# HUBioDataLab/DrugGEN

Hardware: AMD Instinct MI355X
Metric: molecules/sec GAN step (G+D fwd+bwd), N=45 graphs (higher is better)
Workload: dtype f32

## Files before the change

### druggen_amd/csrc/edge_ffn.hip

```cpp
#include "bf16.h"

using namespace dg;

extern "C" size_t dg_edge_ffn_ln_workspace_bytes(int64_t R, int C, int H) {
    const size_t ln = dg_ln_workspace_bytes(R, C);
    const size_t w1 = dg_linear_wgrad_workspace_bytes(R, H, C), w2 = dg_linear_wgrad_workspace_bytes(R, C, H);
    if (!ln || !w1 || !w2) return 0;
    return ((ln + 255) / 256 + (w1 + 255) / 256 + (w2 + 255) / 256) * 256;
}

extern "C" int dg_edge_ffn_ln_fwd(const void* x, const void* w1_packed, const float* b1, const void* w2_packed,
                                  const float* b2, const float* gamma, const float* beta, void* y, void* h,
                                  unsigned* relu_bits, void* pre_ln, float* mean, float* rstd, int64_t R, int C,
                                  int H, float eps, int dtype, dg_stream_t stream) {
    if (!x || !w1_packed || !b1 || !w2_packed || !b2 || !gamma || !beta || !y || !h || !mean || !rstd)
        return fail(DG_E_ARG, "dg_edge_ffn_ln_fwd: null pointer");
    if (C != 128 || H != 384) return fail(DG_E_SHAPE, "dg_edge_ffn_ln_fwd: needs dim 128, hidden 384 (got %d, %d)", C, H);
    int st = dg_row_gemm(x, w1_packed, h, R, C, H, b1, 1, relu_bits, nullptr, nullptr, nullptr, nullptr, nullptr,
                         nullptr, nullptr, 0.f, dtype, stream);
    if (st) return st;
    return dg_row_gemm(h, w2_packed, y, R, H, C, b2, 0, nullptr, nullptr, x, gamma, beta, mean, rstd, pre_ln, eps,
                       dtype, stream);
}

extern "C" int dg_edge_ffn_ln_bwd(const void* x, const void* h, const unsigned* relu_bits, const void* pre_ln,
                                  const float* mean, const float* rstd, const float* gamma,
                                  const void* w1_dgrad_packed, const void* w2_dgrad_packed, const void* dy,
                                  const void* dz_add, void* dz, void* dh, void* dx, float* dgamma, float* dbeta, float* dw1,
                                  float* db1, float* dw2, float* db2, void* workspace, size_t workspace_bytes,
                                  int64_t R, int C, int H, int dtype, dg_stream_t stream) {
    if (!x || !h || !relu_bits || !pre_ln || !mean || !rstd || !gamma || !w1_dgrad_packed || !w2_dgrad_packed ||
        !dz || !dh || !workspace)
        return fail(DG_E_ARG, "dg_edge_ffn_ln_bwd: null pointer");
    if (!dy && dz_add != dz)
        return fail(DG_E_ARG, "dg_edge_ffn_ln_bwd: dy == NULL means dz already holds the LayerNorm input gradient (pass it as dz_add too)");
    if (C != 128 || H != 384) return fail(DG_E_SHAPE, "dg_edge_ffn_ln_bwd: needs dim 128, hidden 384 (got %d, %d)", C, H);
    if (workspace_bytes < dg_edge_ffn_ln_workspace_bytes(R, C, H))
        return fail(DG_E_WORKSPACE, "dg_edge_ffn_ln_bwd: workspace too small");
    int st = 0;
    const size_t lnb = (dg_ln_workspace_bytes(R, C) + 255) / 256 * 256;
    const bool batch = dw2 && dw1;
    if (batch) dg_linear_wgrad_batch_begin();
    if (dy)
        st = dg_ln_residual_bwd_add(pre_ln, nullptr, gamma, mean, rstd, dy, dz_add, dz, dgamma, dbeta, workspace,
                                    lnb, R, C, act_dtype(dtype), stream);
    if (st) {
        if (batch) dg_linear_wgrad_batch_end(stream);
        return st;
    }
    workspace = static_cast<char*>(workspace) + lnb;
    workspace_bytes -= lnb;
    const int dt_h = ffn_h_dtype(dtype), dt_dh = ffn_dh_dtype(dtype);
    st = dg_row_gemm(dz, w2_dgrad_packed, dh, R, C, H, nullptr, 0, nullptr, relu_bits, nullptr, nullptr, nullptr,
                     nullptr, nullptr, nullptr, 0.f, dt_dh, stream);
    if (!st && dx)
        st = dg_row_gemm(dh, w1_dgrad_packed, dx, R, H, C, nullptr, 0, nullptr, nullptr, dz, nullptr, nullptr,
                         nullptr, nullptr, nullptr, 0.f, dt_dh, stream);
    if (st) {
        if (batch) dg_linear_wgrad_batch_end(stream);
        return st;
    }
    if (batch) {
        const size_t w2b = (dg_linear_wgrad_workspace_bytes(R, C, H) + 255) / 256 * 256;
        st = dg_linear_wgrad(dz, nullptr, h, dw2, db2, workspace, w2b, R, C, H, dt_h, stream);
        if (!st)
            st = dg_linear_wgrad(dh, nullptr, x, dw1, db1, static_cast<char*>(workspace) + w2b, workspace_bytes - w2b, R, H, C,
                                 dt_dh, stream);
        const int st2 = dg_linear_wgrad_batch_end(stream);
        return st ? st : st2;
    }
    if (dw2) {
        st = dg_linear_wgrad(dz, nullptr, h, dw2, db2, workspace, workspace_bytes, R, C, H, dt_h, stream);
        if (st) return st;
    }
    if (dw1) {
        st = dg_linear_wgrad(dh, nullptr, x, dw1, db1, workspace, workspace_bytes, R, H, C, dt_dh, stream);
        if (st) return st;
    }
    return 0;
}

namespace {

int ffn_fwd_check(const dg_ffn_fwd_args* a, const char* who) {
    if (!a || !a->x || !a->w1_packed || !a->b1 || !a->w2_packed || !a->b2 || !a->gamma || !a->beta || !a->y || !a->h ||
        !a->mean || !a->rstd)
        return fail(DG_E_ARG, "dg_edge_ffn_ln_fwd_pair: null pointer (%s)", who);
    return 0;
}

int ffn_bwd_phase(const dg_ffn_bwd_args& a, int phase, int C, int H, int dtype, dg_stream_t stream) {
    const int64_t R = a.R;
    const size_t lnb = (dg_ln_workspace_bytes(R, C) + 255) / 256 * 256;
    const size_t w2b = (dg_linear_wgrad_workspace_bytes(R, C, H) + 255) / 256 * 256;
    char* ws = static_cast<char*>(a.workspace);
    switch (phase) {
        case 0:
            if (!a.dy) return 0;
            return dg_ln_residual_bwd_add(a.pre_ln, nullptr, a.gamma, a.mean, a.rstd, a.dy, a.dz_add, a.dz, a.dgamma, a.dbeta, ws,
                                          lnb, R, C, act_dtype(dtype), stream);
        case 1:
            return dg_row_gemm(a.dz, a.w2_dgrad_packed, a.dh, R, C, H, nullptr, 0, nullptr, a.relu_bits, nullptr, nullptr,
                               nullptr, nullptr, nullptr, nullptr, 0.f, ffn_dh_dtype(dtype), stream);
        case 2:
            if (!a.dx) return 0;
            return dg_row_gemm(a.dh, a.w1_dgrad_packed, a.dx, R, H, C, nullptr, 0, nullptr, nullptr, a.dz, nullptr, nullptr,
                               nullptr, nullptr, nullptr, 0.f, ffn_dh_dtype(dtype), stream);
        case 3:
            if (!a.dw2) return 0;
            return dg_linear_wgrad(a.dz, nullptr, a.h, a.dw2, a.db2, ws + lnb, w2b, R, C, H, ffn_h_dtype(dtype), stream);
        default:
            if (!a.dw1) return 0;
            return dg_linear_wgrad(a.dh, nullptr, a.x, a.dw1, a.db1, ws + lnb + w2b, a.workspace_bytes - lnb - w2b, R, H, C,
                                   ffn_dh_dtype(dtype), stream);
    }
}

}

extern "C" int dg_edge_ffn_ln_fwd_pair(const dg_ffn_fwd_args* node, const dg_ffn_fwd_args* edge, int C, int H, int dtype,
                                       dg_stream_t stream) {
    if (int st = ffn_fwd_check(node, "node")) return st;
    if (int st = ffn_fwd_check(edge, "edge")) return st;
    if (C != 128 || H != 384) return fail(DG_E_SHAPE, "dg_edge_ffn_ln_fwd_pair: needs dim 128, hidden 384 (got %d, %d)", C, H);
    const dg_ffn_fwd_args* ps[2] = {node, edge};
    dg_launch_pair_begin();
    int st = 0;
    for (int i = 0; i < 2 && !st; ++i)
        st = dg_row_gemm(ps[i]->x, ps[i]->w1_packed, ps[i]->h, ps[i]->R, C, H, ps[i]->b1, 1, ps[i]->relu_bits, nullptr, nullptr,
                         nullptr, nullptr, nullptr, nullptr, nullptr, 0.f, dtype, stream);
    for (int i = 0; i < 2 && !st; ++i)
        st = dg_row_gemm(ps[i]->h, ps[i]->w2_packed, ps[i]->y, ps[i]->R, H, C, ps[i]->b2, 0, nullptr, nullptr, ps[i]->x,
                         ps[i]->gamma, ps[i]->beta, ps[i]->mean, ps[i]->rstd, ps[i]->pre_ln, ps[i]->eps, dtype, stream);
    const int st2 = dg_launch_pair_end(stream);
    return st ? st : st2;
}

extern "C" int dg_edge_ffn_ln_bwd_pair(const dg_ffn_bwd_args* node, const dg_ffn_bwd_args* edge, int C, int H, int dtype,
                                       dg_stream_t stream) {
    const dg_ffn_bwd_args* ps[2] = {node, edge};
    for (const dg_ffn_bwd_args* a : ps) {
        if (!a || !a->x || !a->h || !a->relu_bits || !a->pre_ln || !a->mean || !a->rstd || !a->gamma || !a->w1_dgrad_packed ||
            !a->w2_dgrad_packed || !a->dz || !a->dh || !a->workspace)
            return fail(DG_E_ARG, "dg_edge_ffn_ln_bwd_pair: null pointer");
        if (!a->dy && a->dz_add != a->dz)
            return fail(DG_E_ARG, "dg_edge_ffn_ln_bwd_pair: dy == NULL means dz already holds the LayerNorm input gradient (pass it as dz_add too)");
        if (a->workspace_bytes < dg_edge_ffn_ln_workspace_bytes(a->R, C, H))
            return fail(DG_E_WORKSPACE, "dg_edge_ffn_ln_bwd_pair: workspace too small");
    }
    if (C != 128 || H != 384) return fail(DG_E_SHAPE, "dg_edge_ffn_ln_bwd_pair: needs dim 128, hidden 384 (got %d, %d)", C, H);
    dg_linear_wgrad_batch_begin();
    dg_launch_pair_begin();
    int st = 0;
    for (int phase = 0; phase < 5 && !st; ++phase)
        for (int i = 0; i < 2 && !st; ++i) st = ffn_bwd_phase(*ps[i], phase, C, H, dtype, stream);
    const int st2 = dg_launch_pair_end(stream);
    const int st3 = dg_linear_wgrad_batch_end(stream);
    return st ? st : (st2 ? st2 : st3);
}
```

### druggen_amd/csrc/row_gemm.hip

```cpp
#include "common.h"
#include "f16_scale.h"
#include "lane_reduce.h"
#include "row_gemm_n384.h"
#include "row_gemm_k384.h"
#include "traversal.h"

#include <cstring>
#include <type_traits>

#ifndef DG_DBG
#define DG_DBG 0
#endif
namespace dg {
namespace {

typedef float f32x16 __attribute__((ext_vector_type(16)));

constexpr int kTR = 64;

struct Epilogue {
    const float* bias;
    const unsigned* mask_bits;
    unsigned* relu_bits;
    const float* residual;
// ... 1117 lines not shown
    return check_launch("dg_row_gemm_ln_bwd");
}

bool reduce_batch_try_add(const float* part, int S, long long n_floats, float* out);

int row_gemm_f32_ln_in(const float* dy, const float* pre, const float* mean, const float* rstd, const float* gamma,
                       const float* packed, float* dz, float* y, float* dgamma, float* dbeta, void* workspace,
                       size_t workspace_bytes, int64_t R, dg_stream_t stream_) {
    if (!dy || !pre || !mean || !rstd || !gamma || !packed || !dz || !y || !workspace)
        return fail(DG_E_ARG, "dg_row_gemm_ln_bwd_in: null pointer");
    if (R < 0) return fail(DG_E_SHAPE, "dg_row_gemm_ln_bwd_in: R = %lld", static_cast<long long>(R));
    if (workspace_bytes < row_gemm_f32_ln_bwd_workspace_bytes()) return fail(DG_E_WORKSPACE, "dg_row_gemm_ln_bwd_in: workspace too small");
    if (R == 0) return 0;
    hipStream_t stream = static_cast<hipStream_t>(stream_);
    Epilogue ep{nullptr, nullptr, nullptr, nullptr, gamma, nullptr, const_cast<float*>(mean), const_cast<float*>(rstd), nullptr, 0.f, 0};
    ep.lna_pre = pre;
    ep.lna_dz = dz;
    ep.lnb_part = static_cast<float*>(workspace);
    const int64_t tiles = (R + kTR - 1) / kTR;
    const int seqs = static_cast<int>(tiles < 256 ? tiles : 256);
    {
        ProfScope prof(R < edge_rows() ? DG_K_ROW_GEMM : DG_K_ROW_GEMM_E_128, stream);
        note_forward(R);
        constexpr int lds = kH3Lds + 4 * 32 * 32 * 4;
        DG_OPT_IN_LDS((&row_gemm_h3_kernel<1, false, false, true>), lds);
        hipLaunchKernelGGL((row_gemm_h3_kernel<1, false, false, true>), dim3(seqs), dim3(512), lds, stream, dy,
                           reinterpret_cast<const f16x8*>(packed), y, R, ep);
    }
    if ((dgamma || dbeta) && !(dgamma && dbeta == dgamma + 128 && reduce_batch_try_add(ep.lnb_part, seqs * 8, 256, dgamma)))
        launch_ln_finish(ep.lnb_part, seqs * 8, 2, 128, dgamma, dbeta, stream);
    return check_launch("dg_row_gemm_ln_bwd_in");
}


int row_gemm_f32_lin3(const float* a, const float* packed, float* y0, float* y1, float* y2, int64_t R, const float* b0,
                      const float* b1, const float* b2, dg_stream_t stream_) {
    if (!a || !packed || !y0 || !y1 || !y2) return fail(DG_E_ARG, "dg_row_gemm_lin3: null pointer");
    if (R < 0) return fail(DG_E_SHAPE, "dg_row_gemm_lin3: negative row count");
    if (R == 0) return 0;
    hipStream_t stream = static_cast<hipStream_t>(stream_);
    Epilogue ep{b0, nullptr, nullptr, nullptr, nullptr, nullptr, nullptr, nullptr, nullptr, 0.f, 0};
    ep.y_alt[0] = y1;
    ep.y_alt[1] = y2;
    ep.bias_alt[0] = b1;
    ep.bias_alt[1] = b2;
    const int64_t tiles = (R + kTR - 1) / kTR;
    const int seqs = static_cast<int>(tiles < 256 ? tiles : 256);
    ProfScope prof(R < edge_rows() ? DG_K_ROW_GEMM : DG_K_ROW_GEMM_E_N384, stream);
    constexpr int lds3 = kH3Lds + 4 * 32 * 32 * 4;
    DG_OPT_IN_LDS((&row_gemm_h3_kernel<3, false, false, false, true>), lds3);
    hipLaunchKernelGGL((row_gemm_h3_kernel<3, false, false, false, true>), dim3(seqs), dim3(512), lds3, stream, a,
                       reinterpret_cast<const f16x8*>(packed), y0, R, ep);
    return check_launch("dg_row_gemm_lin3");
}

int row_gemm_f32_sum3(const float* a0, const float* a1, const float* a2, const float* packed, float* y, int64_t R,
                      const float* residual, dg_stream_t stream_) {
    if (!a0 || !a1 || !a2 || !packed || !y) return fail(DG_E_ARG, "dg_row_gemm_sum3: null pointer");
    if (R < 0) return fail(DG_E_SHAPE, "dg_row_gemm_sum3: negative row count");
    if (R == 0) return 0;
    hipStream_t stream = static_cast<hipStream_t>(stream_);
    Epilogue ep{nullptr, nullptr, nullptr, residual, nullptr, nullptr, nullptr, nullptr, nullptr, 0.f, 0};
    ep.a_alt[0] = a1;
    ep.a_alt[1] = a2;
    const int64_t tiles = (R + kTR - 1) / kTR;
    const int seqs = static_cast<int>(tiles < 256 ? tiles : 256);
// ... 16 lines not shown
```

### druggen_amd/csrc/row_gemm_n384.h

```cpp
#pragma once

#include "common.h"

namespace dg {

size_t row_gemm_n384_mask_words(int64_t R);
int launch_row_gemm_n384(const float* a, const void* packed, void* y, float* yscale, int64_t R, const float* bias, int relu,
                         unsigned* relu_bits, const unsigned* mask_bits, hipStream_t stream, int yfmt = 0, void* ylo = nullptr);
int flush_row_gemm_n384(hipStream_t stream);

}
```

### druggen_amd/csrc/row_gemm_n384.hip

```cpp
#include "common.h"

#include <cstdlib>
#include "row_gemm_n384.h"
#include "lane_reduce.h"
#include "f16_scale.h"
#include "pair.h"
#include "traversal.h"

#ifndef N3_SCHED
#define N3_SCHED 1
#endif
#ifndef N3_DBG
#define N3_DBG 0
#endif
namespace dg {
namespace {

constexpr int kSR = 32;
constexpr int kPlane = 16 * 512;
constexpr int kStage = 2 * kPlane + 128;
constexpr int kOut = kSR * 96 * 16;
constexpr int kOffOut = 2 * kStage;
constexpr int kOffTab = kOffOut + 2 * kOut;
constexpr int kOffBitsIn = kOffTab + 2 * 384 * 4;
constexpr int kOffBitsOut = kOffBitsIn + 2 * 2048;
constexpr int kLds = kOffBitsOut + 2 * 2048;
constexpr int kCons = 8, kProd = 4, kDepth = 3;

struct Epi {
    const float* bias;
    const unsigned* mask_bits;
    unsigned* relu_bits;
    int relu;
    int reverse;
};

struct Prob {
    const float* a;
    const f16x8* packed;
    float* y;
    float* yscale;
    void* ylo;
    int yfmt;
    int64_t R;
    Epi ep;
};

template <int FMT, int MODE, int NP = 3>
__global__ __launch_bounds__(64 * (kCons + kProd)) void row_gemm_n384_kernel(const Prob p0, const Prob p1, const int nb0) {
    constexpr bool H16 = FMT == 1 || FMT == 3, TWO = FMT == 3, H24 = FMT == 2;
    static_assert(NP == 3 || ((NP == 1 || NP == 2) && FMT == 1 && MODE == 2), "reduced products: fp16-plane results of the backward only");
    extern __shared__ __attribute__((aligned(16))) char smem[];
    float* const tab = reinterpret_cast<float*>(smem + kOffTab);
    const int lane = threadIdx.x & 63;
    const int w = __builtin_amdgcn_readfirstlane(threadIdx.x >> 6);
    const bool second = static_cast<int>(blockIdx.x) >= nb0;
    const float* __restrict__ const a = second ? p1.a : p0.a;
    const f16x8* __restrict__ const packed = second ? p1.packed : p0.packed;
    float* __restrict__ const y = second ? p1.y : p0.y;
    float* __restrict__ const yscale = second ? p1.yscale : p0.yscale;
    void* __restrict__ const ylo = second ? p1.ylo : p0.ylo;
    const int64_t R = second ? p1.R : p0.R;
    const Epi ep = second ? p1.ep : p0.ep;
    const int bidx = second ? static_cast<int>(blockIdx.x) - nb0 : static_cast<int>(blockIdx.x);
    const int nblk = second ? static_cast<int>(gridDim.x) - nb0 : nb0;
    const int64_t total = (R + kSR - 1) / kSR;
    const int T = static_cast<int>((total - bidx + nblk - 1) / nblk);
    auto stage_of = [&](int t) {
        const int64_t st = bidx + static_cast<int64_t>(t) * nblk;
        return ep.reverse ? total - 1 - st : st;
    };
    const int TP = (T + kDepth - 1) / kDepth * kDepth;

    if (w >= kCons) {
        __builtin_amdgcn_s_setprio(3);
        const int pt = threadIdx.x - 64 * kCons;
        const int hw = pt >> 5, l32 = pt & 31;
        {
            const float* inv_cs = reinterpret_cast<const float*>(packed + static_cast<size_t>(12) * 8 * 2 * 64);
            for (int i = pt; i < 384; i += 64 * kProd) {
                tab[i] = inv_cs[i];
                tab[384 + i] = ep.bias ? ep.bias[i] : 0.f;
            }
        }
        float4 pf[kDepth][4];
        u32x2 mk[kDepth];
        const unsigned voff = static_cast<unsigned>(hw) * 512u + static_cast<unsigned>(l32) * 16u;
        auto fetch = [&](float4 (&set)[4], u32x2& mword, int t) {
            if (t > T - 1) t = T - 1;
            const __amdgpu_buffer_rsrc_t rmask = __builtin_amdgcn_make_buffer_rsrc(
                const_cast<unsigned*>(ep.mask_bits ? ep.mask_bits + stage_of(t) * 512 : reinterpret_cast<const unsigned*>(a)), 0,
                ep.mask_bits ? 2048 : 0, 0x00020000);
            mword = __builtin_amdgcn_raw_buffer_load_b64(rmask, static_cast<unsigned>(pt) * 8u, 0, 0);
            const int64_t r0 = stage_of(t) * kSR;
            const int64_t left = (R - r0) * 512;
            const __amdgpu_buffer_rsrc_t rsrc = __builtin_amdgcn_make_buffer_rsrc(
                const_cast<float*>(a) + r0 * 128, 0, static_cast<int>(left < (1 << 30) ? left : (1 << 30)), 0x00020000);
            if (N3_DBG & 8) return;
#pragma unroll
            for (int i = 0; i < 4; ++i)
                set[i] = __builtin_bit_cast(float4, __builtin_amdgcn_raw_buffer_load_b128(rsrc, voff, i * 4096, 0));
        };
        const int blk = l32 >> 1;
        const unsigned wbase = static_cast<unsigned>(blk * 512 + (l32 & 1) * 8);
        auto split = [&](float4 (&set)[4], const u32x2& mword, int t) {
// ... 118 lines not shown
                const int64_t left = (R - r0) * 1152;
                const int bytes = ok ? static_cast<int>(left < kSR * 1152 ? left : kSR * 1152) : 0;
                const __amdgpu_buffer_rsrc_t rsrc = __builtin_amdgcn_make_buffer_rsrc(reinterpret_cast<char*>(y) + r0 * 1152, 0, bytes, 0x00020000);
                const unsigned g24 = static_cast<unsigned>(hw) * 1152u + static_cast<unsigned>(l32 ^ hw) * 12u;
                dg_u32x3 pk[12];
#pragma unroll
                for (int i = 0; i < 12; ++i) {
                    const int k = i / 3, qq = i % 3;
                    const float4 v = *reinterpret_cast<const float4*>(ot + ooff + k * 8 * 1536 + qq * 512);
                    pk[i] = pack_f24x4(v.x, v.y, v.z, v.w);
                }
                asm volatile("" : "+v"(pk[0]), "+v"(pk[1]), "+v"(pk[2]), "+v"(pk[3]), "+v"(pk[4]), "+v"(pk[5]), "+v"(pk[6]), "+v"(pk[7]),
                             "+v"(pk[8]), "+v"(pk[9]), "+v"(pk[10]), "+v"(pk[11]));
#pragma unroll
                for (int i = 0; i < 12; ++i) __builtin_amdgcn_raw_buffer_store_b96(pk[i], rsrc, g24, (i / 3) * 8 * 1152 + (i % 3) * 384, 0);
                asm volatile("s_nop 15" ::: "memory");
            } else {
                const int64_t left = (R - r0) * 1536;
                const int bytes = ok ? static_cast<int>(left < kSR * 1536 ? left : kSR * 1536) : 0;
                const __amdgpu_buffer_rsrc_t rsrc = __builtin_amdgcn_make_buffer_rsrc(y + r0 * 384, 0, bytes, 0x00020000);
#pragma unroll
                for (int i = 0; i < 12; ++i) {
                    const int k = i / 3, qq = i % 3;
                    const u32x4 v = *reinterpret_cast<const u32x4*>(ot + ooff + k * 8 * 1536 + qq * 512);
                    __builtin_amdgcn_raw_buffer_store_b128(v, rsrc, goff, k * 8 * 1536 + qq * 512, 0);
                }
            }
            const __amdgpu_buffer_rsrc_t rbits = __builtin_amdgcn_make_buffer_rsrc(
                ep.relu_bits ? ep.relu_bits + stage_of(tc) * 512 : reinterpret_cast<unsigned*>(y), 0, (ok && ep.relu_bits) ? 2048 : 0,
                0x00020000);
            const u32x2 bw = *reinterpret_cast<const u32x2*>(smem + kOffBitsOut + (tc & 1) * 2048 + pt * 8);
            __builtin_amdgcn_raw_buffer_store_b64(bw, rbits, static_cast<unsigned>(pt) * 8u, 0, 0);
        };
        fetch(pf[0], mk[0], 0);
        fetch(pf[1], mk[1], 1);
        fetch(pf[2], mk[2], 2);
        split(pf[0], mk[0], 0);
        fetch(pf[0], mk[0], 3);
        __syncthreads();
        for (int t = 0; t < TP; t += 3) {
            split(pf[1], mk[1], t + 1);
            fetch(pf[1], mk[1], t + 4);
            store_out(t - 1);
            __syncthreads();
            split(pf[2], mk[2], t + 2);
            fetch(pf[2], mk[2], t + 5);
            store_out(t);
            __syncthreads();
            split(pf[0], mk[0], t + 3);
            fetch(pf[0], mk[0], t + 6);
            store_out(t + 1);
            __syncthreads();
        }
        store_out(TP - 1);
        return;
    }

    const int n = lane & 15, kq = lane >> 4;
    f16x8 wf[3][4][NP == 1 ? 1 : 2];
#pragma unroll
    for (int cb = 0; cb < 3; ++cb) {
        const int ch = 48 * w + 16 * cb + n;
        const int tslab = ch >> 5, col = ch & 31;
#pragma unroll
        for (int ks = 0; ks < 4; ++ks)
#pragma unroll
// ... 79 lines not shown
                            newbits |= (v[i] > 0.f ? 1u : 0u) << bit;
                            v[i] = __uint_as_float((__float_as_uint(fmaxf(v[i], 0.f)) & relu_sel) | (__float_as_uint(v[i]) & ~relu_sel));
                            v[i] = (bits >> bit) & 1u ? v[i] : 0.f;
                        }
                    }
                    const int slot = (c0 >> 2) ^ (row & 7);
                    *reinterpret_cast<float4*>(ot + row * 1536 + slot * 16) = make_float4(v[0], v[1], v[2], v[3]);
                }
            }
            *reinterpret_cast<unsigned*>(smem + kOffBitsOut + (t & 1) * 2048 + (w * 64 + lane) * 4) = newbits;
        }
        __syncthreads();
    }
}

}

size_t row_gemm_n384_mask_words(int64_t R) { return static_cast<size_t>((R + kSR - 1) / kSR) * kCons * 64; }

namespace {
struct Pending {
    bool valid = false;
    Prob p;
};
thread_local Pending g_rider;

int mode_of(const Prob& p) {
    if (p.ep.relu && !p.ep.mask_bits) return 1;
    if (!p.ep.relu && p.ep.mask_bits && !p.ep.relu_bits && !p.ep.bias) return 2;
    return 0;
}
bool same_kernel(const Prob& a, const Prob& b) { return a.yfmt == b.yfmt && mode_of(a) == mode_of(b); }

int launch(const Prob& p0, const Prob* p1, hipStream_t stream) {
    const int64_t st0 = (p0.R + kSR - 1) / kSR, st1 = p1 ? (p1->R + kSR - 1) / kSR : 0;
    int nb0, nb1;
    pair_split(st0, st1, 256, &nb0, &nb1);
    const int mode = mode_of(p0);
#define DG_N384_LAUNCH(H16_, MODE_)                                                                                     \
    {                                                                                                                    \
        DG_OPT_IN_LDS((&row_gemm_n384_kernel<H16_, MODE_>), kLds);                                                       \
        hipLaunchKernelGGL((row_gemm_n384_kernel<H16_, MODE_>), dim3(nb0 + nb1), dim3(64 * (kCons + kProd)), kLds, stream, p0, \
                           p1 ? *p1 : p0, nb0);                                                                          \
    }
    const int dh_products = 2;
    if (p0.yfmt == 1) {
        if (mode == 1) DG_N384_LAUNCH(1, 1)
        else if (mode == 2 && dh_products == 2) {
            DG_OPT_IN_LDS((&row_gemm_n384_kernel<1, 2, 2>), kLds);
            hipLaunchKernelGGL((row_gemm_n384_kernel<1, 2, 2>), dim3(nb0 + nb1), dim3(64 * (kCons + kProd)), kLds, stream, p0,
                               p1 ? *p1 : p0, nb0);
        } else if (mode == 2 && dh_products == 1) {
            DG_OPT_IN_LDS((&row_gemm_n384_kernel<1, 2, 1>), kLds);
            hipLaunchKernelGGL((row_gemm_n384_kernel<1, 2, 1>), dim3(nb0 + nb1), dim3(64 * (kCons + kProd)), kLds, stream, p0,
                               p1 ? *p1 : p0, nb0);
        } else if (mode == 2) DG_N384_LAUNCH(1, 2)
        else DG_N384_LAUNCH(1, 0)
    } else if (p0.yfmt == 3) {
        if (mode == 1) DG_N384_LAUNCH(3, 1)
        else if (mode == 2) DG_N384_LAUNCH(3, 2)
        else DG_N384_LAUNCH(3, 0)
    } else if (p0.yfmt == 2) {
        if (mode == 1) DG_N384_LAUNCH(2, 1)
        else if (mode == 2) DG_N384_LAUNCH(2, 2)
        else DG_N384_LAUNCH(2, 0)
    } else {
        if (mode == 1) DG_N384_LAUNCH(0, 1)
        else if (mode == 2) DG_N384_LAUNCH(0, 2)
        else DG_N384_LAUNCH(0, 0)
    }
#undef DG_N384_LAUNCH
    return 0;
}
}

int flush_row_gemm_n384(hipStream_t stream) {
    if (!g_rider.valid) return 0;
    g_rider.valid = false;
    return launch(g_rider.p, nullptr, stream);
}

int launch_row_gemm_n384(const float* a, const void* packed, void* y, float* yscale, int64_t R, const float* bias, int relu,
                         unsigned* relu_bits, const unsigned* mask_bits, hipStream_t stream, int yfmt, void* ylo) {
    if ((yfmt == 1 || yfmt == 3) != (yscale != nullptr)) return fail(DG_E_ARG, "row_gemm_n384: row scales go with the fp16 planes (yfmt 1, 3)");
    if ((yfmt == 3) != (ylo != nullptr)) return fail(DG_E_ARG, "row_gemm_n384: the lo plane goes with yfmt 3");
    const Prob p{a, static_cast<const f16x8*>(packed), static_cast<float*>(y), yscale, ylo, yfmt, R,
                 Epi{bias, mask_bits, relu_bits, relu, take_direction(R)}};
    if (pair_mode() && !g_rider.valid && R <= kRiderMaxRows) {
        g_rider.valid = true;
        g_rider.p = p;
        return 0;
    }
    if (g_rider.valid) {
        g_rider.valid = false;
        if (same_kernel(p, g_rider.p)) return launch(p, &g_rider.p, stream);
        if (int st = launch(g_rider.p, nullptr, stream)) return st;
    }
    return launch(p, nullptr, stream);
}

}
```

### druggen_amd/functional/_runtime.py

```python
from __future__ import annotations

import contextlib
import threading
import weakref

import torch

from .. import _lib
from ..options import options


_traffic = {}


def traffic_reset() -> None:
    _traffic.clear()


def traffic_bytes(kernel: str) -> int:
    return _traffic.get(kernel, 0)


def _account(kernel: str, nbytes: int, flops: int = 0, floor: int = -1) -> None:
    _traffic[kernel] = _traffic.get(kernel, 0) + nbytes
# ... 60 lines not shown
    if adt == torch.float32:
        mode = hidden_storage()
        if mode in ("f16", "f24"):
            return _lib.F32_H16 if mode == "f16" else _lib.F32_H24
        if hidden_forward_storage(long_rows) == "split":
            return _lib.F32_H32
    return _lib.DTYPES[adt]


def _hidden_code_bwd(adt) -> int:
    if adt == torch.float32:
        mode = hidden_storage()
        if mode in ("f16", "dh16"):
            return _lib.F32_H16
        if mode in ("f24", "dh24"):
            return _lib.F32_H24
    return _lib.DTYPES[adt]


def _ffn_bwd_codes(h, adt, R: int, H: int):
    if _is_h16(h):
        code = _hidden_code_of(h, R, H)
        if code == _lib.F32_H32:
            return _lib.F32_H32_DH16, _lib.F32_H16
        return code, code
    dh_code = _hidden_code_bwd(adt)
    if dh_code == _lib.F32_H16 and hidden_storage() == "dh16":
        dh_code = _lib.F32_H24
    if dh_code == _lib.F32_H16:
        return _lib.F32_DH16, dh_code
    if dh_code == _lib.F32_H24:
        return _lib.F32_DH24, dh_code
    return _lib.DTYPES[adt], _lib.DTYPES[adt]


def _hidden_empty(R: int, H: int, adt, code: int, device):
    if code in _lib.HIDDEN_CODES:
        return torch.empty(int(_lib.load().dg_hidden_bytes(R, H, code)), dtype=torch.uint8, device=device)
    return torch.empty(R, H, dtype=adt, device=device)


def _hrow_bytes(code: int, es: int, H: int) -> int:
    if code == _lib.F32_H32:
        return 4 * H + 4
    return 2 * H + 4 if code == _lib.F32_H16 else (3 * H if code == _lib.F32_H24 else es * H)


def _is_h16(t) -> bool:
    return t is not None and t.dtype == torch.uint8


def _hptr(t):
    return t.data_ptr() if _is_h16(t) else _lib.ptr(t)


def _hidden_code_of(buf, R: int, H: int = 384) -> int:
    if buf.numel() == R * H * 3:
        return _lib.F32_H24
    plane = (R * H * 2 + 255) // 256 * 256
    return _lib.F32_H32 if buf.numel() == 2 * plane + 4 * R else _lib.F32_H16


def hidden_to_float(buf, R: int, H: int = 384):
    if _hidden_code_of(buf, R, H) == _lib.F32_H24:
        b = buf.view(R * H, 3).to(torch.int32)
        bits = (b[:, 0] << 8) | (b[:, 1] << 16) | (b[:, 2] << 24)
# ... 239 lines not shown
```

### druggen_amd/functional/ffn.py

```python
from __future__ import annotations

import ctypes

import torch
from torch.autograd import Function
from torch.autograd.function import once_differentiable

from .. import _lib
from ..options import options
from ._runtime import (_account, _alias_outputs_enabled, _c, _ffn_bwd_codes, _gemm_key, _hidden_code, _hidden_code_of,
                       _hidden_empty, hidden_storage, _hptr, _hrow_bytes, in_second_order_forward, _inputs_only, _is_h16,
                       _long_rows, PackCache, _pair_launches, _scratch, _weight_alias, _wgrad_key)
from .layernorm import ln_residual
from .dense import _double_backward_fallback, _join_alias_grads, linear, _ln_bwd2_rows, packed_weight, row_gemm, _wgrad_many


def _fused_ffn_enabled() -> bool:
    return options.ffn_bf16 == "fused"


def _composite_ffn_ln(x, w1, b1, w2, b2, gamma, beta, eps):
    return ln_residual(x, linear(torch.relu(linear(x, w1, b1)), w2, b2), gamma, beta, eps)


_ffn_f32_pack_cache = PackCache(1024)


def _ffn_packed_f32(w1, w2):
    def make(w1, w2):
        lib = _lib.load()
        packed = torch.empty(int(lib.dg_ffn_f32_packed_bytes()), dtype=torch.uint8, device=w1.device)
        _lib.launch("dg_ffn_f32_pack", w1, _lib.fptr(_c(w1.detach())), _lib.fptr(_c(w2.detach())), packed.data_ptr())
        return packed
    return _ffn_f32_pack_cache.get((w1, w2), (), make)


def set_fused_ffn_f32(on: bool) -> None:
    options.ffn_f32 = "fused" if on else "unfused"


def fused_ffn_f32_supported(x2, w1, w2, long_rows: bool = False) -> bool:
    return (options.ffn_f32 == "fused" and x2.is_cuda and x2.dtype == torch.float32 and tuple(w1.shape) == (384, 128)
            and tuple(w2.shape) == (128, 384) and hidden_storage() == "dh16" and not long_rows)
# ... 62 lines not shown
    return probs


def _ffn_saved(args, p):
    return (*args, p["h"], p["mean"], p["rstd"], p["pre"], p["bits"])


def _ffn_bwd_inputs(saved, needs, dy, dpre):
    x, w1, b1, w2, b2, gamma, beta, h, mean, rstd, pre, bits = saved
    want_w = needs[1] and not _inputs_only()
    want_aff = (needs[5] or needs[6]) and not _inputs_only()
    if dy is None and (dpre is None or torch.is_grad_enabled()):
        dy = torch.zeros_like(pre)
    return [x, w1, b1, w2, b2, gamma, h, mean, rstd, pre, bits, dy, dpre, needs[0], want_w, want_aff]


def _ffn_bwd_problem(x, w1, b1, w2, b2, gamma, h, mean, rstd, pre, bits, dy, dz_add, want_x, want_w, want_aff=None):
    H, C = w1.shape
    adt = pre.dtype
    rows = lambda t: _c(t if t.dtype == adt else t.to(adt)).reshape(-1, C)
    p = dict(x=x, x2=_c(x).reshape(-1, C), w1=w1, w2=w2, gamma=gamma, h=h, mean=mean, rstd=rstd, pre=pre, bits=bits,
             R=pre.shape[0], C=C, H=H, want_x=want_x, want_w=want_w, want_aff=want_w if want_aff is None else want_aff,
             had_add=dz_add is not None)
    if dy is None:
        p["dy2"] = None
        p["dz"] = p["dz_add"] = rows(dz_add)
    else:
        p["dy2"] = rows(dy)
        p["dz_add"] = None if dz_add is None else rows(dz_add)
        p["dz"] = None
    return p


def _ffn_bwd_account(p, code, dh_code):
    R, C, H = p["R"], p["C"], p["H"]
    es = p["pre"].element_size()
    if p["dy2"] is not None:
        _account("ln_bwd", es * R * C * (4 if p["dz_add"] is not None else 3))
    hb = _hrow_bytes(_hidden_code_of(p["h"], R, H) if _is_h16(p["h"]) else _lib.dt(p["pre"]), es, H)
    dhb = _hrow_bytes(dh_code, es, H)
    _account(_gemm_key(R, C, H), R * (es * C + dhb), 2 * R * C * H)
    if p["dx"] is not None:
        _account(_gemm_key(R, H, C), R * (dhb + es * 2 * C), 2 * R * C * H)
    if p["want_w"]:
        _account(_wgrad_key(R, C, H), R * (es * C + (2 * H + 4 if code == _lib.F32_H32_DH16 else hb)), 2 * R * C * H)
        _account(_wgrad_key(R, H, C), R * (es * C + dhb), 2 * R * C * H)


def _ffn_bwd(ctx, args):
    lib = _lib.load()
    probs = [_ffn_bwd_problem(*args[k:k + 16]) for k in range(0, len(args), 16)]
    p0 = probs[0]
    ref = p0["pre"]
    adt, dev = ref.dtype, ref.device
    code, dh_code = _ffn_bwd_codes(p0["h"], adt, p0["R"], p0["H"])
    cargs = []
    for i, p in enumerate(probs):
        R, C, H = p["R"], p["C"], p["H"]
        p["dgamma"] = p["dbeta"] = None
        if p["dy2"] is not None:
            p["dz"] = torch.empty(R, C, dtype=adt, device=dev)
            if p["want_aff"]:
                p["dgamma"], p["dbeta"] = torch.empty(2, p["gamma"].numel(), dtype=p["gamma"].dtype, device=dev).unbind(0)
        p["dh"] = _hidden_empty(R, H, adt, dh_code, dev)
        p["dx"] = torch.empty(R, C, dtype=adt, device=dev) if p["want_x"] else None
        p["dw1"] = p["db1"] = p["dw2"] = p["db2"] = None
        if p["want_w"]:
            p["dw1"], p["dw2"] = torch.empty_like(p["w1"]), torch.empty_like(p["w2"])
            p["db1"] = torch.empty(H, dtype=torch.float32, device=dev)
            p["db2"] = torch.empty(C, dtype=torch.float32, device=dev)
        ws = _scratch(ref, int(lib.dg_edge_ffn_ln_workspace_bytes(R, C, H)), "ffn" if len(probs) == 1 else f"ffn_pair{i}")
        cargs.append((
            _lib.ptr(p["x2"]), _hptr(p["h"]), p["bits"].data_ptr(), _lib.ptr(p["pre"]), _lib.ptr(p["mean"]),
            _lib.ptr(p["rstd"]), _lib.fptr(_c(p["gamma"])), packed_weight(p["w1"], 1, adt).data_ptr(),
            packed_weight(p["w2"], 1, adt).data_ptr(), _lib.ptr(p["dy2"]), _lib.ptr(p["dz_add"]), _lib.ptr(p["dz"]),
            _hptr(p["dh"]), _lib.ptr(p["dx"]), _lib.ptr(p["dgamma"]), _lib.ptr(p["dbeta"]), _lib.ptr(p["dw1"]),
            _lib.ptr(p["db1"]), _lib.ptr(p["dw2"]), _lib.ptr(p["db2"]), ws.data_ptr(), ws.numel(), R))
    if len(probs) == 1:
        _lib.launch("dg_edge_ffn_ln_bwd", ref, *cargs[0], p0["C"], p0["H"], code)
    else:
        _lib.launch("dg_edge_ffn_ln_bwd_pair", ref, *(ctypes.byref(_lib.FFNBwdArgs(*c)) for c in cargs), p0["C"], p0["H"],
                    code)
    saved, outs = [], []
    for p in probs:
        _ffn_bwd_account(p, code, dh_code)
        saved += [p["x"], p["w1"], p["w2"], p["gamma"], p["h"], p["mean"], p["rstd"], p["pre"], p["bits"], p["dy2"], p["dz"], p["dh"]]
        outs += [None if p["dx"] is None else p["dx"].view(p["x"].shape), p["dw1"], p["db1"], p["dw2"], p["db2"],
                 p["dgamma"], p["dbeta"]]
    ctx.save_for_backward(*saved)
    ctx.had_add = tuple(p["had_add"] for p in probs)
    ctx.set_materialize_grads(False)
    return tuple(outs)


def _ffn_bwd2(ctx, t):
    n = len(t) // 7
    if any(g is not None for k in range(n) for g in t[7 * k + 1:7 * k + 7]):
        raise RuntimeError("ffn_ln: second-order terms through parameter gradients are not implemented")
    sv = ctx.saved_tensors
    probs = []
    for i in range(n):
        t_dx = t[7 * i]
        if t_dx is None:
            probs.append(None)
            continue
        if ctx.had_add[i]:
            raise RuntimeError("ffn_ln: third-order differentiation is not implemented")
        x, w1, w2, gamma, h, mean, rstd, pre, bits, dy2, dz, dh = sv[12 * i:12 * i + 12]
        H, C = w1.shape
        adt = pre.dtype
        probs.append(dict(w1=w1, w2=w2, gamma=gamma, mean=mean, rstd=rstd, pre=pre, bits=bits, dy2=dy2, dz=dz, dh=dh, C=C, H=H,
                          t_dx=t_dx, t=_c(t_dx if t_dx.dtype == adt else t_dx.to(adt)).reshape(-1, C), gw1=None, gw2=None))
    live = [p for p in probs if p is not None]
    if not live:
        return (None,) * (16 * n)
    p0 = live[0]
    ref = p0["pre"]
    pw = lambda w_, m_: packed_weight(w_, m_, ref.dtype)
# ... 214 lines not shown
```

Baseline: 4966.

## Fuse LayerNorm-residual backward into the N=384 row GEMM prologue for edge FFN

After: 5014, median of 6. No clear change (+1.0%).

```diff
diff --git a/druggen_amd/csrc/edge_ffn.hip b/druggen_amd/csrc/edge_ffn.hip
--- a/druggen_amd/csrc/edge_ffn.hip
+++ b/druggen_amd/csrc/edge_ffn.hip
@@ -1,9 +1,32 @@
 #include "bf16.h"
+#include "row_gemm_n384.h"
 
 using namespace dg;
 
+namespace {
+
+bool ffn_ln_fused(const void* dy, int64_t R, int dtype) {
+    return dy && R >= edge_rows() && act_dtype(dtype) == DG_DTYPE_F32 && ffn_dh_dtype(dtype) == DG_DTYPE_F32_H16;
+}
+
+size_t ffn_ln_part_bytes(int64_t R, int C) {
+    const size_t a = dg_ln_workspace_bytes(R, C), b = row_gemm_f32_n384_ln_in_workspace_bytes(R);
+    return ((a > b ? a : b) + 255) / 256 * 256;
+}
+
+int ffn_ln_gemm_fused(const void* pre_ln, const float* mean, const float* rstd, const float* gamma, const void* w2_dgrad_packed,
+                      const unsigned* relu_bits, const void* dy, const void* dz_add, void* dz, void* dh, float* dgamma, float* dbeta,
+                      void* workspace, size_t lnb, int64_t R, dg_stream_t stream) {
+    float* dh_scale = reinterpret_cast<float*>(static_cast<char*>(dh) + hidden_scale_offset(R, 384));
+    return row_gemm_f32_n384_ln_in(static_cast<const float*>(dy), static_cast<const float*>(pre_ln), mean, rstd, gamma,
+                                   static_cast<const float*>(dz_add), static_cast<const float*>(w2_dgrad_packed), relu_bits,
+                                   static_cast<float*>(dz), dh, dh_scale, dgamma, dbeta, workspace, lnb, R, stream);
+}
+
+}
+
 extern "C" size_t dg_edge_ffn_ln_workspace_bytes(int64_t R, int C, int H) {
-    const size_t ln = dg_ln_workspace_bytes(R, C);
+    const size_t ln = dg_ln_workspace_bytes(R, C) ? ffn_ln_part_bytes(R, C) : 0;
     const size_t w1 = dg_linear_wgrad_workspace_bytes(R, H, C), w2 = dg_linear_wgrad_workspace_bytes(R, C, H);
     if (!ln || !w1 || !w2) return 0;
     return ((ln + 255) / 256 + (w1 + 255) / 256 + (w2 + 255) / 256) * 256;
@@ -38,21 +61,27 @@
     if (workspace_bytes < dg_edge_ffn_ln_workspace_bytes(R, C, H))
         return fail(DG_E_WORKSPACE, "dg_edge_ffn_ln_bwd: workspace too small");
     int st = 0;
-    const size_t lnb = (dg_ln_workspace_bytes(R, C) + 255) / 256 * 256;
+    const size_t lnb = ffn_ln_part_bytes(R, C);
+    const bool fused = ffn_ln_fused(dy, R, dtype);
     const bool batch = dw2 && dw1;
     if (batch) dg_linear_wgrad_batch_begin();
-    if (dy)
+    if (dy && !fused)
         st = dg_ln_residual_bwd_add(pre_ln, nullptr, gamma, mean, rstd, dy, dz_add, dz, dgamma, dbeta, workspace,
                                     lnb, R, C, act_dtype(dtype), stream);
     if (st) {
         if (batch) dg_linear_wgrad_batch_end(stream);
         return st;
     }
+    void* const ws_ln = workspace;
     workspace = static_cast<char*>(workspace) + lnb;
     workspace_bytes -= lnb;
     const int dt_h = ffn_h_dtype(dtype), dt_dh = ffn_dh_dtype(dtype);
-    st = dg_row_gemm(dz, w2_dgrad_packed, dh, R, C, H, nullptr, 0, nullptr, relu_bits, nullptr, nullptr, nullptr,
-                     nullptr, nullptr, nullptr, 0.f, dt_dh, stream);
+    if (fused)
+        st = ffn_ln_gemm_fused(pre_ln, mean, rstd, gamma, w2_dgrad_packed, relu_bits, dy, dz_add, dz, dh, dgamma, dbeta,
+                               ws_ln, lnb, R, stream);
+    else
+        st = dg_row_gemm(dz, w2_dgrad_packed, dh, R, C, H, nullptr, 0, nullptr, relu_bits, nullptr, nullptr, nullptr,
+                         nullptr, nullptr, nullptr, 0.f, dt_dh, stream);
     if (!st && dx)
         st = dg_row_gemm(dh, w1_dgrad_packed, dx, R, H, C, nullptr, 0, nullptr, nullptr, dz, nullptr, nullptr,
                          nullptr, nullptr, nullptr, 0.f, dt_dh, stream);
@@ -89,17 +118,21 @@
     return 0;
 }
 
-int ffn_bwd_phase(const dg_ffn_bwd_args& a, int phase, int C, int H, int dtype, dg_stream_t stream) {
+int ffn_bwd_phase(const dg_ffn_bwd_args& a, int phase, int C, int H, int dtype, dg_stream_t stream, bool fuse) {
     const int64_t R = a.R;
-    const size_t lnb = (dg_ln_workspace_bytes(R, C) + 255) / 256 * 256;
+    const size_t lnb = ffn_ln_part_bytes(R, C);
+    const bool fused = fuse && ffn_ln_fused(a.dy, R, dtype);
     const size_t w2b = (dg_linear_wgrad_workspace_bytes(R, C, H) + 255) / 256 * 256;
     char* ws = static_cast<char*>(a.workspace);
     switch (phase) {
         case 0:
-            if (!a.dy) return 0;
+            if (!a.dy || fused) return 0;
             return dg_ln_residual_bwd_add(a.pre_ln, nullptr, a.gamma, a.mean, a.rstd, a.dy, a.dz_add, a.dz, a.dgamma, a.dbeta, ws,
                                           lnb, R, C, act_dtype(dtype), stream);
         case 1:
+            if (fused)
+                return ffn_ln_gemm_fused(a.pre_ln, a.mean, a.rstd, a.gamma, a.w2_dgrad_packed, a.relu_bits, a.dy, a.dz_add, a.dz, a.dh,
+                                         a.dgamma, a.dbeta, ws, lnb, R, stream);
             return dg_row_gemm(a.dz, a.w2_dgrad_packed, a.dh, R, C, H, nullptr, 0, nullptr, a.relu_bits, nullptr, nullptr,
                                nullptr, nullptr, nullptr, nullptr, 0.f, ffn_dh_dtype(dtype), stream);
         case 2:
@@ -153,7 +186,7 @@
     dg_launch_pair_begin();
     int st = 0;
     for (int phase = 0; phase < 5 && !st; ++phase)
-        for (int i = 0; i < 2 && !st; ++i) st = ffn_bwd_phase(*ps[i], phase, C, H, dtype, stream);
+        for (int i = 0; i < 2 && !st; ++i) st = ffn_bwd_phase(*ps[i], phase, C, H, dtype, stream, i == 1);
     const int st2 = dg_launch_pair_end(stream);
     const int st3 = dg_linear_wgrad_batch_end(stream);
     return st ? st : (st2 ? st2 : st3);
diff --git a/druggen_amd/csrc/row_gemm.hip b/druggen_amd/csrc/row_gemm.hip
--- a/druggen_amd/csrc/row_gemm.hip
+++ b/druggen_amd/csrc/row_gemm.hip
@@ -1173,6 +1173,29 @@
     return check_launch("dg_row_gemm_ln_bwd_in");
 }
 
+size_t row_gemm_f32_n384_ln_in_workspace_bytes(int64_t R) { return static_cast<size_t>(row_gemm_n384_ln_max_parts(R)) * 256 * sizeof(float); }
+
+int row_gemm_f32_n384_ln_in(const float* dy, const float* pre, const float* mean, const float* rstd, const float* gamma,
+                            const float* dz_add, const float* packed, const unsigned* mask_bits, float* dz, void* dh, float* dh_scale,
+                            float* dgamma, float* dbeta, void* workspace, size_t workspace_bytes, int64_t R, dg_stream_t stream_) {
+    if (!dy || !pre || !mean || !rstd || !gamma || !packed || !mask_bits || !dz || !dh || !dh_scale || !workspace)
+        return fail(DG_E_ARG, "dg_edge_ffn_ln_bwd: null pointer");
+    if (R < 1) return fail(DG_E_SHAPE, "dg_edge_ffn_ln_bwd: R = %lld", static_cast<long long>(R));
+    if (workspace_bytes < row_gemm_f32_n384_ln_in_workspace_bytes(R)) return fail(DG_E_WORKSPACE, "dg_edge_ffn_ln_bwd: workspace too small");
+    hipStream_t stream = static_cast<hipStream_t>(stream_);
+    N384LnIn ln;
+    ln.pre = pre; ln.mean = mean; ln.rstd = rstd; ln.gamma = gamma; ln.add = dz_add; ln.dz = dz;
+    ln.part = static_cast<float*>(workspace);
+    int parts = 0;
+    {
+        ProfScope prof(R < edge_rows() ? DG_K_ROW_GEMM : DG_K_ROW_GEMM_E_N384, stream);
+        if (int st = launch_row_gemm_n384_ln(dy, packed, dh, dh_scale, R, mask_bits, ln, &parts, stream)) return st;
+    }
+    if ((dgamma || dbeta) && !(dgamma && dbeta == dgamma + 128 && reduce_batch_try_add(ln.part, parts, 256, dgamma)))
+        launch_ln_finish(ln.part, parts, 2, 128, dgamma, dbeta, stream);
+    return check_launch("dg_edge_ffn_ln_bwd");
+}
+
 
 int row_gemm_f32_lin3(const float* a, const float* packed, float* y0, float* y1, float* y2, int64_t R, const float* b0,
                       const float* b1, const float* b2, dg_stream_t stream_) {
diff --git a/druggen_amd/csrc/row_gemm_n384.h b/druggen_amd/csrc/row_gemm_n384.h
--- a/druggen_amd/csrc/row_gemm_n384.h
+++ b/druggen_amd/csrc/row_gemm_n384.h
@@ -7,6 +7,25 @@
 size_t row_gemm_n384_mask_words(int64_t R);
 int launch_row_gemm_n384(const float* a, const void* packed, void* y, float* yscale, int64_t R, const float* bias, int relu,
                          unsigned* relu_bits, const unsigned* mask_bits, hipStream_t stream, int yfmt = 0, void* ylo = nullptr);
+struct N384LnIn {
+    const float* pre = nullptr;
+    const float* mean = nullptr;
+    const float* rstd = nullptr;
+    const float* gamma = nullptr;
+    const float* add = nullptr;
+    float* dz = nullptr;
+    float* part = nullptr;
+};
+inline int row_gemm_n384_ln_max_parts(int64_t R) {
+    const int64_t st = (R + 31) / 32;
+    return static_cast<int>(st < 256 ? st : 256) * 8;
+}
+int launch_row_gemm_n384_ln(const float* dy, const void* packed, void* y, float* yscale, int64_t R, const unsigned* mask_bits,
+                            const N384LnIn& ln, int* parts, hipStream_t stream);
+size_t row_gemm_f32_n384_ln_in_workspace_bytes(int64_t R);
+int row_gemm_f32_n384_ln_in(const float* dy, const float* pre, const float* mean, const float* rstd, const float* gamma,
+                            const float* dz_add, const float* packed, const unsigned* mask_bits, float* dz, void* dh, float* dh_scale,
+                            float* dgamma, float* dbeta, void* workspace, size_t workspace_bytes, int64_t R, dg_stream_t stream);
 int flush_row_gemm_n384(hipStream_t stream);
 
 }
diff --git a/druggen_amd/csrc/row_gemm_n384.hip b/druggen_amd/csrc/row_gemm_n384.hip
--- a/druggen_amd/csrc/row_gemm_n384.hip
+++ b/druggen_amd/csrc/row_gemm_n384.hip
@@ -44,12 +44,14 @@
     int yfmt;
     int64_t R;
     Epi ep;
+    N384LnIn ln;
 };
 
-template <int FMT, int MODE, int NP = 3>
+template <int FMT, int MODE, int NP = 3, bool LNA = false>
 __global__ __launch_bounds__(64 * (kCons + kProd)) void row_gemm_n384_kernel(const Prob p0, const Prob p1, const int nb0) {
     constexpr bool H16 = FMT == 1 || FMT == 3, TWO = FMT == 3, H24 = FMT == 2;
     static_assert(NP == 3 || ((NP == 1 || NP == 2) && FMT == 1 && MODE == 2), "reduced products: fp16-plane results of the backward only");
+    static_assert(!LNA || (FMT == 1 && MODE == 2 && NP == 2), "LayerNorm-backward prologue: dh = (dz W2) * m into the fp16 plane");
     extern __shared__ __attribute__((aligned(16))) char smem[];
     float* const tab = reinterpret_cast<float*>(smem + kOffTab);
     const int lane = threadIdx.x & 63;
@@ -62,6 +64,8 @@
     void* __restrict__ const ylo = second ? p1.ylo : p0.ylo;
     const int64_t R = second ? p1.R : p0.R;
     const Epi ep = second ? p1.ep : p0.ep;
+    const N384LnIn ln = second ? p1.ln : p0.ln;
+    const bool lna = LNA && ln.pre != nullptr;
     const int bidx = second ? static_cast<int>(blockIdx.x) - nb0 : static_cast<int>(blockIdx.x);
     const int nblk = second ? static_cast<int>(gridDim.x) - nb0 : nb0;
     const int64_t total = (R + kSR - 1) / kSR;
@@ -70,7 +74,8 @@
         const int64_t st = bidx + static_cast<int64_t>(t) * nblk;
         return ep.reverse ? total - 1 - st : st;
     };
-    const int TP = (T + kDepth - 1) / kDepth * kDepth;
+    const int depth = lna ? 2 : kDepth;
+    const int TP = (T + depth - 1) / depth * depth;
 
     if (w >= kCons) {
         __builtin_amdgcn_s_setprio(3);
@@ -255,6 +260,94 @@
             const u32x2 bw = *reinterpret_cast<const u32x2*>(smem + kOffBitsOut + (tc & 1) * 2048 + pt * 8);
             __builtin_amdgcn_raw_buffer_store_b64(bw, rbits, static_cast<unsigned>(pt) * 8u, 0, 0);
         };
+        if constexpr (LNA) {
+            if (lna) {
+                float4 prr[4], zad[4];
+                float st = 0.f;
+                const float4 gam = ld4(ln.gamma + l32 * 4);
+                float4 dgam = f4(0.f), dbet = f4(0.f);
+                const bool upper = (lane & 32) != 0;
+                auto fetch_pre = [&](int t) {
+                    if (t > T - 1) t = T - 1;
+                    const int64_t r0 = stage_of(t) * kSR;
+                    const int64_t left = (R - r0) * 512;
+                    const int range = static_cast<int>(left < (1 << 30) ? left : (1 << 30));
+                    const __amdgpu_buffer_rsrc_t rp = __builtin_amdgcn_make_buffer_rsrc(const_cast<float*>(ln.pre) + r0 * 128, 0, range, 0x00020000);
+                    const __amdgpu_buffer_rsrc_t ra = __builtin_amdgcn_make_buffer_rsrc(
+                        const_cast<float*>(ln.add ? ln.add : ln.pre) + r0 * 128, 0, ln.add ? range : 0, 0x00020000);
+#pragma unroll
+                    for (int i = 0; i < 4; ++i) prr[i] = __builtin_bit_cast(float4, __builtin_amdgcn_raw_buffer_load_b128(rp, voff, i * 4096, 0));
+#pragma unroll
+                    for (int i = 0; i < 4; ++i) zad[i] = __builtin_bit_cast(float4, __builtin_amdgcn_raw_buffer_load_b128(ra, voff, i * 4096, 0));
+                    int64_t row = r0 + hw + 8 * (l32 & 3);
+                    if (row > R - 1) row = R - 1;
+                    st = (l32 & 4) ? ln.rstd[row] : ln.mean[row];
+                };
+                auto ln_split = [&](float4 (&set)[4], const u32x2& mword, int t) {
+                    const bool ok = t < T;
+                    const float live = ok ? 1.f : 0.f;
+                    const int tc = ok ? t : T - 1;
+                    const int64_t r0 = stage_of(tc) * kSR;
+                    const int64_t left = R - r0;
+                    const int rows = ok ? static_cast<int>(left < kSR ? left : kSR) : 0;
+                    const __amdgpu_buffer_rsrc_t rdz = __builtin_amdgcn_make_buffer_rsrc(ln.dz + r0 * 128, 0, rows * 512, 0x00020000);
+                    const int sti = __float_as_int(st);
+#pragma unroll
+                    for (int i = 0; i < 4; ++i) {
+                        const int mu0 = __builtin_amdgcn_readlane(sti, i), mu1 = __builtin_amdgcn_readlane(sti, 32 + i);
+                        const int rs0 = __builtin_amdgcn_readlane(sti, 4 + i), rs1 = __builtin_amdgcn_readlane(sti, 36 + i);
+                        const float mu = __int_as_float(upper ? mu1 : mu0), rs = __int_as_float(upper ? rs1 : rs0);
+                        const float4 v = set[i];
+                        const float4 xh = rs * (prr[i] - f4(mu));
+                        const float4 u = v * gam;
+                        const float c1 = half_wave_total_readlane((u.x + u.y) + (u.z + u.w), upper) * (1.0f / 128.0f);
+                        const float c2 = half_wave_total_readlane((u.x * xh.x + u.y * xh.y) + (u.z * xh.z + u.w * xh.w), upper) * (1.0f / 128.0f);
+                        float4 dz = rs * (u - f4(c1) - c2 * xh);
+                        const float4 vm = live * v;
+                        dgam = fma4(vm, xh, dgam);
+                        dbet += vm;
+                        asm volatile("" : "+v"(dz.x), "+v"(dz.y), "+v"(dz.z), "+v"(dz.w));
+                        if (ln.add) dz += zad[i];
+                        set[i] = dz;
+                    }
+                    asm volatile("" : "+v"(set[0].x), "+v"(set[0].y), "+v"(set[0].z), "+v"(set[0].w), "+v"(set[1].x), "+v"(set[1].y),
+                                 "+v"(set[1].z), "+v"(set[1].w));
+                    asm volatile("" : "+v"(set[2].x), "+v"(set[2].y), "+v"(set[2].z), "+v"(set[2].w), "+v"(set[3].x), "+v"(set[3].y),
+                                 "+v"(set[3].z), "+v"(set[3].w));
+#pragma unroll
+                    for (int i = 0; i < 4; ++i)
+                        __builtin_amdgcn_raw_buffer_store_b128(__builtin_bit_cast(u32x4, set[i]), rdz, voff, i * 4096, 0);
+                    asm volatile("s_nop 15" ::: "memory");
+                    __builtin_amdgcn_sched_barrier(0);
+                    split(set, mword, t);
+                    __builtin_amdgcn_sched_barrier(0);
+                };
+                fetch(pf[0], mk[0], 0);
+                fetch_pre(0);
+                fetch(pf[1], mk[1], 1);
+                ln_split(pf[0], mk[0], 0);
+                fetch(pf[0], mk[0], 2);
+                fetch_pre(1);
+                __syncthreads();
+                for (int t = 0; t < TP; t += 2) {
+                    ln_split(pf[1], mk[1], t + 1);
+                    fetch(pf[1], mk[1], t + 3);
+                    store_out(t - 1);
+                    fetch_pre(t + 2);
+                    __syncthreads();
+                    ln_split(pf[0], mk[0], t + 2);
+                    fetch(pf[0], mk[0], t + 4);
+                    store_out(t);
+                    fetch_pre(t + 3);
+                    __syncthreads();
+                }
+                store_out(TP - 1);
+                float* pp = ln.part + (static_cast<size_t>(bidx) * 8 + hw) * 256 + l32 * 4;
+                st4(pp, dgam);
+                st4(pp + 128, dbet);
+                return;
+            }
+        }
         fetch(pf[0], mk[0], 0);
         fetch(pf[1], mk[1], 1);
         fetch(pf[2], mk[2], 2);
@@ -400,11 +493,18 @@
 }
 bool same_kernel(const Prob& a, const Prob& b) { return a.yfmt == b.yfmt && mode_of(a) == mode_of(b); }
 
-int launch(const Prob& p0, const Prob* p1, hipStream_t stream) {
+int launch(const Prob& p0, const Prob* p1, hipStream_t stream, int* nb0_out = nullptr) {
     const int64_t st0 = (p0.R + kSR - 1) / kSR, st1 = p1 ? (p1->R + kSR - 1) / kSR : 0;
     int nb0, nb1;
     pair_split(st0, st1, 256, &nb0, &nb1);
+    if (nb0_out) *nb0_out = nb0;
     const int mode = mode_of(p0);
+    if (p0.ln.pre) {
+        DG_OPT_IN_LDS((&row_gemm_n384_kernel<1, 2, 2, true>), kLds);
+        hipLaunchKernelGGL((row_gemm_n384_kernel<1, 2, 2, true>), dim3(nb0 + nb1), dim3(64 * (kCons + kProd)), kLds, stream, p0,
+                           p1 ? *p1 : p0, nb0);
+        return 0;
+    }
 #define DG_N384_LAUNCH(H16_, MODE_)                                                                                     \
     {                                                                                                                    \
         DG_OPT_IN_LDS((&row_gemm_n384_kernel<H16_, MODE_>), kLds);                                                       \
@@ -453,7 +553,7 @@
     if ((yfmt == 1 || yfmt == 3) != (yscale != nullptr)) return fail(DG_E_ARG, "row_gemm_n384: row scales go with the fp16 planes (yfmt 1, 3)");
     if ((yfmt == 3) != (ylo != nullptr)) return fail(DG_E_ARG, "row_gemm_n384: the lo plane goes with yfmt 3");
     const Prob p{a, static_cast<const f16x8*>(packed), static_cast<float*>(y), yscale, ylo, yfmt, R,
-                 Epi{bias, mask_bits, relu_bits, relu, take_direction(R)}};
+                 Epi{bias, mask_bits, relu_bits, relu, take_direction(R)}, N384LnIn{}};
     if (pair_mode() && !g_rider.valid && R <= kRiderMaxRows) {
         g_rider.valid = true;
         g_rider.p = p;
@@ -467,4 +567,23 @@
     return launch(p, nullptr, stream);
 }
 
-}
+int launch_row_gemm_n384_ln(const float* dy, const void* packed, void* y, float* yscale, int64_t R, const unsigned* mask_bits,
+                            const N384LnIn& ln, int* parts, hipStream_t stream) {
+    if (!yscale || !mask_bits || !ln.pre || !ln.mean || !ln.rstd || !ln.gamma || !ln.dz || !ln.part)
+        return fail(DG_E_ARG, "row_gemm_n384: the LayerNorm-backward prologue needs the fp16-plane result, a ReLU mask and the LayerNorm's operands");
+    note_forward(R);
+    const Prob p{dy, static_cast<const f16x8*>(packed), static_cast<float*>(y), yscale, nullptr, 1, R,
+                 Epi{nullptr, mask_bits, nullptr, 0, 0}, ln};
+    const Prob* rider = nullptr;
+    if (g_rider.valid) {
+        g_rider.valid = false;
+        if (same_kernel(p, g_rider.p)) rider = &g_rider.p;
+        else if (int st = launch(g_rider.p, nullptr, stream)) return st;
+    }
+    int nb0 = 0;
+    const int st = launch(p, rider, stream, &nb0);
+    *parts = nb0 * 8;
+    return st;
+}
+
+}
diff --git a/druggen_amd/functional/_runtime.py b/druggen_amd/functional/_runtime.py
--- a/druggen_amd/functional/_runtime.py
+++ b/druggen_amd/functional/_runtime.py
@@ -116,6 +116,10 @@
     if dh_code == _lib.F32_H24:
         return _lib.F32_DH24, dh_code
     return _lib.DTYPES[adt], _lib.DTYPES[adt]
+
+
+def _ffn_ln_in_gemm(has_dy: bool, R: int, adt, dh_code: int) -> bool:
+    return has_dy and R >= _lib.edge_rows() and adt == torch.float32 and dh_code == _lib.F32_H16
 
 
 def _hidden_empty(R: int, H: int, adt, code: int, device):
diff --git a/druggen_amd/functional/ffn.py b/druggen_amd/functional/ffn.py
--- a/druggen_amd/functional/ffn.py
+++ b/druggen_amd/functional/ffn.py
@@ -8,7 +8,7 @@
 
 from .. import _lib
 from ..options import options
-from ._runtime import (_account, _alias_outputs_enabled, _c, _ffn_bwd_codes, _gemm_key, _hidden_code, _hidden_code_of,
+from ._runtime import (_account, _alias_outputs_enabled, _c, _ffn_bwd_codes, _ffn_ln_in_gemm, _gemm_key, _hidden_code, _hidden_code_of,
                        _hidden_empty, hidden_storage, _hptr, _hrow_bytes, in_second_order_forward, _inputs_only, _is_h16,
                        _long_rows, PackCache, _pair_launches, _scratch, _weight_alias, _wgrad_key)
 from .layernorm import ln_residual
@@ -137,14 +137,15 @@
     return p
 
 
-def _ffn_bwd_account(p, code, dh_code):
+def _ffn_bwd_account(p, code, dh_code, may_fuse=True):
     R, C, H = p["R"], p["C"], p["H"]
     es = p["pre"].element_size()
+    fused = may_fuse and _ffn_ln_in_gemm(p["dy2"] is not None, R, p["pre"].dtype, dh_code)
     if p["dy2"] is not None:
-        _account("ln_bwd", es * R * C * (4 if p["dz_add"] is not None else 3))
+        _account(_gemm_key(R, C, H) if fused else "ln_bwd", es * R * C * (4 if p["dz_add"] is not None else 3))
     hb = _hrow_bytes(_hidden_code_of(p["h"], R, H) if _is_h16(p["h"]) else _lib.dt(p["pre"]), es, H)
     dhb = _hrow_bytes(dh_code, es, H)
-    _account(_gemm_key(R, C, H), R * (es * C + dhb), 2 * R * C * H)
+    _account(_gemm_key(R, C, H), R * ((0 if fused else es * C) + dhb), 2 * R * C * H)
     if p["dx"] is not None:
         _account(_gemm_key(R, H, C), R * (dhb + es * 2 * C), 2 * R * C * H)
     if p["want_w"]:
@@ -187,8 +188,8 @@
         _lib.launch("dg_edge_ffn_ln_bwd_pair", ref, *(ctypes.byref(_lib.FFNBwdArgs(*c)) for c in cargs), p0["C"], p0["H"],
                     code)
     saved, outs = [], []
-    for p in probs:
-        _ffn_bwd_account(p, code, dh_code)
+    for i, p in enumerate(probs):
+        _ffn_bwd_account(p, code, dh_code, may_fuse=i == len(probs) - 1)
         saved += [p["x"], p["w1"], p["w2"], p["gamma"], p["h"], p["mean"], p["rstd"], p["pre"], p["bits"], p["dy2"], p["dz"], p["dh"]]
         outs += [None if p["dx"] is None else p["dx"].view(p["x"].shape), p["dw1"], p["db1"], p["dw2"], p["db2"],
                  p["dgamma"], p["dbeta"]]
```
